# SvenGronauer/phoenix-drone-simulation

Measured on AMD Instinct MI355X. Metric: env-steps/sec, higher is better.
Workload: dtype f32; 1 GPU; DroneHoverSimpleEnv-v0, 1048576 envs per GPU lockstep, fp32, observation noise off, thrust noise 0, domain randomisation -1, auto-reset on, action ring [64,N,4] = hover+0.0 + 0.1*N(0,1); envs_per_gpu=1048576, obs_dim=42, bytes_per_env_step=346, parallelism=env-shard x1, no data-path collective

## Files before the change

phoenix-drone-simulation_amd/csrc/pds_api.hip:

```cpp
#include <hip/hip_runtime.h>

#include <cmath>
#include <cstdarg>
#include <cstdio>
#include <cstdlib>
#include <cstring>
#include <new>
#include <utility>
#include <vector>

#include "pds_reset.h"
#include "pds_collect_args.h"
#include "pds_evaluate_args.h"
#include "pds_evaluate_hist_args.h"
#include "pds_simopt.h"

namespace pds {

struct FieldArgs {
  DevState st;
  Consts k;
  void *user;
  long long n;
  int field;
  int task;
  int set;
// ... 182 lines not shown
  if (i >= n) return;
  const uint32_t c = st.ctr[i];
  if (ctr_oh(c) != 0u) return;
  const WaveClock ck = st.clk[i / kWave];
  const RngKey now{seed_lo, seed_hi, ck.x, ck.y};
  const float4 q0 = st.s0[i], q1 = st.s1[i], q2 = st.s2[i];
  const EnvRegs e{q0.x, q0.y, q0.z, q0.w, q1.x, q1.y, q1.z, q1.w, q2.x, q2.y, q2.z, q2.w};
  NoisyObs o;
  regen_kept_obs(k, (uint32_t)(env_id_base + (unsigned long long)i), now, ctr_step(c) == 0u, e, o);
  st.oh0[i] = make_float4(o.x, o.y, o.z, o.qx);
  st.oh1[i] = make_float4(o.qy, o.qz, o.qw, o.vx);
  st.oh2[i] = make_float2(o.vy, o.vz);
  st.ctr[i] = c | kCtrOhBit;
}


}

using namespace pds;

struct pds_handle {
  pds_config cfg;
  DevState st;
  Consts k;
  LaunchFlags flags;
  int force_tile;
  float2 *d_circle_ref;
  void *slab;
  float4 *lat_buf;
  unsigned long long *d_count;
  unsigned long long *d_stamps;
  void *eval_sink;
  int obs_dim;
  int num_cus;
  uint64_t tick;
  bool was_reset;
  bool after_evaluate;
  char err[512];
};

struct DeviceGuard {
  int prev = -1;
  bool switched = false;
  hipError_t err = hipSuccess;
  explicit DeviceGuard(int dev) {
    err = hipGetDevice(&prev);
    if (err == hipSuccess && prev != dev) {
      err = hipSetDevice(dev);
      switched = err == hipSuccess;
    }
  }
  ~DeviceGuard() {
// ... 13 lines not shown

static thread_local char g_create_err[512] = "";

#define PDS_HIP(h, call)                                                                        \
  do {                                                                                          \
    hipError_t e_ = (call);                                                                     \
    if (e_ != hipSuccess) return fail(h, PDS_EHIP, "%s failed: %s", #call, hipGetErrorString(e_)); \
  } while (0)

static int materialize_kept_obs(pds_handle *h, hipStream_t s) {
  if (!(h->flags.on && !h->flags.hold)) return PDS_OK;
  const long long n = h->cfg.num_envs;
  hipLaunchKernelGGL(pds::materialize_oh_kernel, dim3((unsigned)((n + kBlock - 1) / kBlock)), dim3(kBlock), 0, s, h->st, h->k, n,
                     (unsigned long long)h->cfg.env_id_base, (uint32_t)h->cfg.seed, (uint32_t)(h->cfg.seed >> 32));
  PDS_HIP(h, hipGetLastError());
  return PDS_OK;
}

extern "C" int pds_version(void) { return PDS_VERSION; }

extern "C" int pds_default_config(int task, pds_config *c) {
  if (!c || task < 0 || task > 2) return PDS_EINVAL;
  memset(c, 0, sizeof(*c));
  c->struct_size = (int32_t)sizeof(pds_config);
  c->task = task;
  c->num_envs = 1;
  c->env_id_base = 0;
  c->seed = 0;
  c->device = 0;
  c->use_motor_dynamics = 0;
// ... 189 lines not shown
  h->flags.ctrl = cfg->control_mode;
  h->flags.lat = lat_steps > 0;
  h->flags.hold = h->k.obs_rate != 1;
  h->flags.half_tile = false;
  if (const char *ft = getenv("PDS_FORCE_TILE")) h->force_tile = (ft[0] == 'h') ? 1 : ((ft[0] == 'f') ? 2 : 0);
  const size_t n = (size_t)cfg->num_envs;
  const size_t ntiles = (n + kWave - 1) / kWave;
  const LaunchFlags &f = h->flags;
  DeviceGuard guard(cfg->device);
  hipError_t e = guard.err;
  if (e == hipSuccess) {
    hipDeviceProp_t prop;
    e = hipGetDeviceProperties(&prop, cfg->device);
    h->num_cus = (e == hipSuccess && prop.multiProcessorCount > 0) ? prop.multiProcessorCount : 256;
  }
  std::vector<std::pair<void **, size_t>> req;
  auto alloc = [&](void **p, size_t bytes) { req.emplace_back(p, bytes); };
  alloc((void **)&h->st.s0, n * 16); alloc((void **)&h->st.s1, n * 16); alloc((void **)&h->st.s2, n * 16);
  alloc((void **)&h->st.hist[0], n * 16); alloc((void **)&h->st.hist[1], n * 16);
  alloc((void **)&h->st.ctr, n * 4);
  alloc((void **)&h->st.clk, ntiles * sizeof(WaveClock));
  alloc((void **)&h->d_count, 256);
  if (f.motor) alloc((void **)&h->st.mx, n * 16);
  if (f.dr) { alloc((void **)&h->st.par0, n * 16); alloc((void **)&h->st.par1, n * 8); }
  if (f.dr && f.motor) { alloc((void **)&h->st.mA, n * 16); alloc((void **)&h->st.mK, n * 16); }
  if (f.tn) alloc((void **)&h->st.ou, n * 16);
  if (f.on) {
    alloc((void **)&h->st.nz0, n * 16); alloc((void **)&h->st.nz1, n * 8);
    alloc((void **)&h->st.oh0, n * 16); alloc((void **)&h->st.oh1, n * 16); alloc((void **)&h->st.oh2, n * 8);
  }
// ... 69 lines not shown
  if (!h) return 0;
  DeviceGuard guard(h->cfg.device);
  WaveClock c;
  if (hipStreamSynchronize((hipStream_t)stream) == hipSuccess &&
      hipMemcpy(&c, h->st.clk, sizeof(c), hipMemcpyDeviceToHost) == hipSuccess)
    h->tick = ((uint64_t)c.y << 32) | c.x;
  return h->tick;
}

extern "C" int pds_set_tick(pds_handle *h, uint64_t tick) {
  if (!h) return PDS_EINVAL;
  DeviceGuard guard(h->cfg.device);
  PDS_HIP(h, guard.err);
  PDS_HIP(h, hipDeviceSynchronize());
  if (const int rc = materialize_kept_obs(h, 0)) return rc;
  const long long ntiles = (h->cfg.num_envs + kWave - 1) / kWave;
  hipLaunchKernelGGL(clock_fill_kernel, dim3((unsigned)((ntiles + 255) / 256)), dim3(256), 0, 0, h->st.clk, ntiles,
                     (unsigned long long)tick, 1);
  PDS_HIP(h, hipGetLastError());
  PDS_HIP(h, hipDeviceSynchronize());
  h->tick = tick;
  return PDS_OK;
}

extern "C" int pds_set_latency(pds_handle *h, double latency) {
  if (!h) return PDS_EINVAL;
  if (h->flags.ge && h->flags.ctrl != 0) return fail(h, PDS_EUNSUPPORTED, "use_latency with the ground-effect extension: control_mode PWM only");
  int steps = 0;
  if (!(latency < h->cfg.time_step)) {
    steps = (int)(latency / h->cfg.time_step);
    if (steps < 1) return fail(h, PDS_EINVAL, "latency %g: buf_size 0 (the reference asserts buf_size > 0)", latency);
    if (steps > kMaxLatSteps) return fail(h, PDS_EUNSUPPORTED, "latency %g s = %d steps (limit %d)", latency, steps, kMaxLatSteps);
  }
  DeviceGuard guard(h->cfg.device);
  PDS_HIP(h, guard.err);
  PDS_HIP(h, hipDeviceSynchronize());
  if (steps > 0) {
    const int rc = ensure_latency_buffer(h);
    if (rc != PDS_OK) return rc;
  }
  h->cfg.latency = latency;
  h->cfg.use_latency = steps > 0;
  h->flags.lat = steps > 0;
  set_latency_consts(h->k, steps, h->cfg.aggregate_phy_steps);
  if (steps > 0) {
    const long long n = h->cfg.num_envs;
    hipLaunchKernelGGL(latency_clear_kernel, dim3((unsigned)((n + 255) / 256)), dim3(256), 0, 0, h->st, n, kMaxLatSteps);
    PDS_HIP(h, hipGetLastError());
    PDS_HIP(h, hipDeviceSynchronize());
  }
  return PDS_OK;
}

extern "C" int pds_simopt_latency_steps(const pds_handle *h, double latency) {
  if (!h) return PDS_EINVAL;
// ... 16 lines not shown
  if (max_lat_steps > kMaxLatSteps)
    return fail(h, PDS_EUNSUPPORTED, "a candidate's latency is %d time steps (limit %d): nothing was evaluated", max_lat_steps,
                kMaxLatSteps);
  if (P < 1 || M < 1 || T < 2 || pre_steps < 0 || max_lat_steps < 0)
    return fail(h, PDS_EINVAL, "pds_simopt_evaluate: P %lld, M %lld, T %d, pre_steps %d, max_lat_steps %d", (long long)P,
                (long long)M, T, pre_steps, max_lat_steps);
  if (M > (1 << 24) || P > (1 << 24) || P * ((M + kWave - 1) / kWave) > (int64_t)1 << 32)
    return fail(h, PDS_EINVAL, "pds_simopt_evaluate: P %lld x M %lld is beyond one launch: shard the candidates", (long long)P,
                (long long)M);
  if (!d_params || !d_lat_steps || !d_actions || !d_obs || !d_loss || !d_score || (pre_steps > 0 && !d_pre_inputs))
    return fail(h, PDS_EINVAL, "pds_simopt_evaluate: null pointer");
  if (((uintptr_t)d_actions | (uintptr_t)d_obs | (uintptr_t)d_pre_inputs) & 15u)
    return fail(h, PDS_EINVAL, "pds_simopt_evaluate: the data set arrays must be 16-byte aligned");
  DeviceGuard guard(h->cfg.device);
  PDS_HIP(h, guard.err);
  SimoptArgs a;
  a.k = h->k;
  a.time_step = h->cfg.time_step;
  a.G = 9.81;
  a.gamma = gamma;
  a.params = d_params;
  a.lat_steps = d_lat_steps;
  a.acts = reinterpret_cast<const float4 *>(d_actions);
  a.obs = reinterpret_cast<const float4 *>(d_obs);
  a.pre = reinterpret_cast<const float4 *>(d_pre_inputs);
  a.P = (int)P; a.M = (int)M; a.T = T; a.pre_steps = pre_steps;
  a.loss = d_loss; a.score = d_score; a.sim_obs = d_sim_obs;
  launch_simopt(a, (hipStream_t)stream);
  PDS_HIP(h, hipGetLastError());
  return PDS_OK;
// ... 63 lines not shown
    else if (task == PDS_TASK_CIRCLE) launch_circle(kind, lf, grid, s, a);
    else launch_takeoff(kind, lf, grid, s, a);
  }
}

static int do_reset(pds_handle *h, const uint8_t *d_mask, const float *d_samples, float *d_obs, void *stream) {
  if (!h) return PDS_EINVAL;
  DeviceGuard guard(h->cfg.device);
  PDS_HIP(h, guard.err);
  if (d_mask != nullptr && h->after_evaluate)
    return fail(h, PDS_EINVAL, "pds_reset with a mask after pds_evaluate_policies: reset every env first (d_mask = NULL)");
  StepArgs a;
  base_args(h, a);
  a.mask = d_mask; a.samples = d_samples; a.obs = d_obs;
  const dim3 grid((unsigned)((a.n + kBlock - 1) / kBlock));
  if (d_mask != nullptr)
    if (const int rc = materialize_kept_obs(h, (hipStream_t)stream)) return rc;
  launch_family(h, kLaunchReset, h->flags, grid, (hipStream_t)stream, a);
  PDS_HIP(h, hipGetLastError());
  h->tick += 1;
  h->was_reset = true;
  h->after_evaluate = false;
  return PDS_OK;
}

extern "C" int pds_reset(pds_handle *h, const uint8_t *d_mask, float *d_obs, void *stream) {
  return do_reset(h, d_mask, nullptr, d_obs, stream);
}

extern "C" int pds_reset_from_samples(pds_handle *h, const uint8_t *d_mask, const float *d_samples,
                                      float *d_obs, void *stream) {
  if (h && !d_samples) return fail(h, PDS_EINVAL, "pds_reset_from_samples: d_samples is NULL");
  return do_reset(h, d_mask, d_samples, d_obs, stream);
}

static int check_step_pointers(pds_handle *h, const float *d_actions, float *d_obs, float *d_reward, uint8_t *d_terminated,
                               uint8_t *d_truncated, float *d_cost) {
// ... 13 lines not shown
  DeviceGuard guard(h->cfg.device);
  PDS_HIP(h, guard.err);
  StepArgs a;
  base_args(h, a);
  a.actions = reinterpret_cast<const float4 *>(d_actions);
  a.obs = d_obs; a.reward = d_reward; a.term = d_terminated; a.trunc = d_truncated; a.cost = d_cost;
  a.final_obs = d_final_obs;
  a.noise = d_variates;
  const dim3 grid((unsigned)((a.n + kBlock - 1) / kBlock));
  LaunchFlags lf = h->flags;
  const bool merged = !lf.on && !lf.lat && !(lf.motor && lf.dr) && h->cfg.task != PDS_TASK_TAKEOFF && h->cfg.auto_reset;
  const unsigned cus = (unsigned)h->num_cus;
  lf.half_tile = grid.x > (unsigned)kFullTileBlocksPerCU * cus * (256 / kBlock) && grid.x <= (merged ? 5u : 8u) * cus * (256 / kBlock);
  if (h->force_tile) lf.half_tile = h->force_tile == 1;
  if (lf.on || lf.lat) lf.half_tile = false;
  launch_family(h, kLaunchStep, lf, grid, (hipStream_t)stream, a);
  PDS_HIP(h, hipGetLastError());
  h->tick += 1;
  return PDS_OK;
}

extern "C" int pds_step(pds_handle *h, const float *d_actions, float *d_obs, float *d_reward,
                        uint8_t *d_terminated, uint8_t *d_truncated, float *d_cost, float *d_final_obs,
                        void *stream) {
  return pds_step_with_variates(h, d_actions, nullptr, d_obs, d_reward, d_terminated, d_truncated, d_cost,
                                d_final_obs, stream);
}

extern "C" int pds_step_k(pds_handle *h, int k_steps, const float *d_actions, float *d_obs, float *d_reward,
                          uint8_t *d_terminated, uint8_t *d_truncated, float *d_cost, float *d_final_obs, void *stream) {
  if (!h) return PDS_EINVAL;
  if (k_steps < 1) return fail(h, PDS_EINVAL, "pds_step_k: k_steps %d", k_steps);
// ... 9 lines not shown
    }
    return PDS_OK;
  }
  DeviceGuard guard(h->cfg.device);
  PDS_HIP(h, guard.err);
  StepArgs a;
  base_args(h, a);
  a.actions = reinterpret_cast<const float4 *>(d_actions);
  a.obs = d_obs; a.reward = d_reward; a.term = d_terminated; a.trunc = d_truncated; a.cost = d_cost;
  a.final_obs = d_final_obs;
  a.k_steps = k_steps;
  const dim3 grid((unsigned)((a.n + kBlock - 1) / kBlock));
  LaunchFlags lf = h->flags;
  lf.half_tile = false;
  if (const int rc = materialize_kept_obs(h, (hipStream_t)stream)) return rc;
  launch_family(h, kLaunchStepK, lf, grid, (hipStream_t)stream, a);
  PDS_HIP(h, hipGetLastError());
  h->tick += (uint64_t)k_steps;
  return PDS_OK;
}

extern "C" int pds_field_width(int field) {
  switch (field) {
    case PDS_F_POS: case PDS_F_RPY: case PDS_F_VEL: case PDS_F_OMEGA: case PDS_F_GYRO_BIAS: case PDS_F_GYRO_LPF: return 3;
    case PDS_F_QUAT: case PDS_F_MOTOR_X: case PDS_F_LAST_ACTION: case PDS_F_PREV_ACTION: case PDS_F_MOTOR_A:
    case PDS_F_MOTOR_K: case PDS_F_OU: return 4;
    case PDS_F_STEP_COUNT: case PDS_F_QUAT_SIGN: case PDS_F_REF_OFFSET: case PDS_F_ACTION_IDX: return 1;
    case PDS_F_PARAMS: return 6;
    case PDS_F_NOISY_OBS: return 10;
    case PDS_F_PID: return 12;
// ... 27 lines not shown
  ra.s.reward = d_rew_buf; ra.s.term = d_term_buf; ra.s.trunc = d_trunc_buf; ra.s.cost = d_cost_buf;
  ra.s.final_obs = nullptr;
  ra.s.k_steps = T;
  ra.pi = *pi;
  ra.mean = d_mean; ra.stdv = d_std; ra.eps = eps; ra.log_std = d_log_std;
  ra.seed = seed; ra.call_base = reinterpret_cast<const unsigned long long *>(d_call_base); ra.call_offset = call_offset;
  ra.deterministic = deterministic; ra.T = T;
  ra.act_buf = d_act_buf; ra.logp_buf = d_logp_buf;
  ra.ep_ret = d_ep_ret; ra.ep_len = d_ep_len; ra.stats = d_stats;
}
template <class Launch>
static int launch_rollout(pds_handle *h, const char *fn, int T, void *stream, Launch launch) {
  DeviceGuard guard(h->cfg.device);
  PDS_HIP(h, guard.err);
  if (const int rc = materialize_kept_obs(h, (hipStream_t)stream)) return rc;
  const dim3 grid((unsigned)((h->cfg.num_envs + kWave - 1) / kWave));
  if (!launch(grid, (hipStream_t)stream)) return fail(h, PDS_EHIP, "%s: its _supported() rule and the launchers disagree", fn);
  PDS_HIP(h, hipGetLastError());
  h->tick += (uint64_t)T;
  return PDS_OK;
}

extern "C" int pds_rollout(pds_handle *h, int T, const pds_mlp *pi, const pds_mlp *vf, const float *d_mean, const float *d_std,
                           float eps, const float *d_log_std, uint64_t seed, const uint64_t *d_call_base, uint64_t call_offset,
                           int deterministic, float *d_obs_buf, float *d_act_buf, float *d_logp_buf, float *d_val_buf,
                           float *d_rew_buf, uint8_t *d_term_buf, uint8_t *d_trunc_buf, float *d_cost_buf, float *d_fval_buf,
                           float *d_last_val, float *d_ep_ret, float *d_ep_len, float *d_stats, void *stream) {
  if (!h) return PDS_EINVAL;
  if (T < 1) return fail(h, PDS_EINVAL, "pds_rollout: T %d", T);
  const bool any_null = !pi || !vf || !d_log_std || !d_obs_buf || !d_act_buf || !d_logp_buf || !d_val_buf || !d_rew_buf ||
// ... 383 lines not shown
}

static int do_field(pds_handle *h, int field, void *d_ptr, int set, void *stream) {
  if (!h) return PDS_EINVAL;
  if (!d_ptr || pds_field_width(field) < 0) return fail(h, PDS_EINVAL, "bad field %d or NULL pointer", field);
  if (set && field == PDS_F_QUAT) return fail(h, PDS_EINVAL, "PDS_F_QUAT is derived (set PDS_F_RPY / PDS_F_QUAT_SIGN)");
  DeviceGuard guard(h->cfg.device);
  PDS_HIP(h, guard.err);
  FieldArgs a;
  memset(&a, 0, sizeof(a));
  a.st = h->st; a.k = h->k; a.user = d_ptr; a.n = h->cfg.num_envs; a.field = field; a.task = h->cfg.task; a.set = set;
  a.has_motor = h->flags.motor; a.has_dr = h->flags.dr; a.has_tn = h->flags.tn; a.has_on = h->flags.on; a.ctrl = h->flags.ctrl;
  a.regen_obs = h->flags.on && !h->flags.hold;
  if (set && field != PDS_F_NOISY_OBS)
    if (const int rc = materialize_kept_obs(h, (hipStream_t)stream)) return rc;
  a.env_id_base = (unsigned long long)h->cfg.env_id_base;
  a.seed_lo = (uint32_t)h->cfg.seed; a.seed_hi = (uint32_t)(h->cfg.seed >> 32);
  const dim3 grid((unsigned)((a.n + kBlock - 1) / kBlock));
  hipLaunchKernelGGL(field_kernel, grid, dim3(kBlock), 0, (hipStream_t)stream, a);
  PDS_HIP(h, hipGetLastError());
  if (set && !h->after_evaluate) h->was_reset = true;
  return PDS_OK;
}

extern "C" int pds_count_nonfinite(pds_handle *h, int64_t *count, void *stream) {
  if (!h || !count) return PDS_EINVAL;
  DeviceGuard guard(h->cfg.device);
  PDS_HIP(h, guard.err);
  hipStream_t s = (hipStream_t)stream;
  PDS_HIP(h, hipMemsetAsync(h->d_count, 0, sizeof(*h->d_count), s));
  const long long n = h->cfg.num_envs;
  hipLaunchKernelGGL(nonfinite_kernel, dim3((unsigned)((n + 255) / 256)), dim3(256), 0, s, h->st, n, h->d_count);
  PDS_HIP(h, hipGetLastError());
  unsigned long long host = 0;
  PDS_HIP(h, hipMemcpyAsync(&host, h->d_count, sizeof(host), hipMemcpyDeviceToHost, s));
  PDS_HIP(h, hipStreamSynchronize(s));
  *count = (int64_t)host;
  return PDS_OK;
}

extern "C" int pds_get_state(pds_handle *h, int field, void *d_out, void *stream) { return do_field(h, field, d_out, 0, stream); }
extern "C" int pds_set_state(pds_handle *h, int field, const void *d_in, void *stream) { return do_field(h, field, const_cast<void *>(d_in), 1, stream); }

template <int ROUNDS>
// ... 77 lines not shown
```

phoenix-drone-simulation_amd/csrc/pds_step.h:

```cpp
#pragma once
#include <type_traits>
#include "pds_reset.h"
#include "pds_physics.h"

namespace pds {

template <int D>
constexpr int tile_stride() {
  return (D % 8 == 0) ? D + 4 : D;
}

template <int HW>
constexpr int park_stride() {
  return (HW % 4 == 0) ? ((HW / 4) % 2 == 1 ? HW : HW + 4) : (HW % 2 == 1 ? HW : HW + 1);
}

template <int N>
PDS_DEV void lds_store_row(float *dst, const float *src) {
  static_assert(N % 4 == 0, "float4 rows");
#pragma unroll
  for (int j = 0; j < N / 4; ++j)
    reinterpret_cast<float4 *>(dst)[j] = make_float4(src[4 * j], src[4 * j + 1], src[4 * j + 2], src[4 * j + 3]);
}

template <class V>
constexpr bool heavy_variant() { return V::MOTOR || V::DR || V::TN || V::ON || V::CTRL != 0 || V::LAT; }

template <class V>
constexpr bool saddr_variant() { return heavy_variant<V>(); }
template <class V>
constexpr bool park_variant() { return heavy_variant<V>(); }
template <class V>
using Idx = EnvIdxT<saddr_variant<V>()>;

template <class V>
constexpr bool regen_obs_variant() { return V::ON && !V::HOLD && !V::OH_STORED; }
template <class V>
constexpr bool flags_oh_variant() { return V::ON && !V::HOLD && V::OH_STORED; }

template <int D, int TR, bool SADDR>
PDS_DEV void flush_tile(const float *tile, float *gdst, int rows, int lane) {
  constexpr int TS = tile_stride<D>();
  const bool fast = rows == TR && (reinterpret_cast<uintptr_t>(gdst) & 15u) == 0;
  if constexpr (TS == D) {
    if (fast) {
      constexpr int NV = TR * D / 4;
      const float4 *src = reinterpret_cast<const float4 *>(tile);
      float4 *dst = reinterpret_cast<float4 *>(gdst);
// ... 130 lines not shown
  if constexpr (regen_obs_variant<V>()) {
    const uint32_t env_id = (uint32_t)(a.env_id_base + (unsigned long long)ix.wb) + ix.lc;
    regen_kept_obs(a.k, env_id, rk, ctr_step(S.ctr) == 0u, S.e, S.oh);
    const bool stored = ctr_oh(S.ctr) != 0u;
    if (__ballot(stored) != 0ull) {
      if (stored) {
        const float4 o0 = *at(a.st.oh0, ix), o1 = *at(a.st.oh1, ix);
        const float2 o2 = *at(a.st.oh2, ix);
        S.oh = NoisyObs{o0.x, o0.y, o0.z, o0.w, o1.x, o1.y, o1.z, o1.w, o2.x, o2.y};
      }
    }
  }
}

template <class V>
PDS_DEV void store_state(const StepArgs &a, const Idx<V> i_, int new_parity, const EnvState &S, bool both) {
  const EnvRegs &e = S.e;
  Idx<V> i = fresh<3>(i_);
  st_store4(at(a.st.s0, i), make_float4(e.px, e.py, e.pz, e.vx));
  st_store4(at(a.st.s1, i), make_float4(e.vy, e.vz, e.roll, e.pitch));
  st_store4(at(a.st.s2, i), make_float4(e.yaw, e.wx, e.wy, e.wz));
  st_store4(at(a.st.hist[new_parity], i), S.h1);
  *at(a.st.ctr, i) = flags_oh_variant<V>() ? (S.ctr | kCtrOhBit) : S.ctr;
  if (V::MOTOR) *at(a.st.mx, i) = make_float4(S.xm[0], S.xm[1], S.xm[2], S.xm[3]);
  if (V::TN) *at(a.st.ou, i) = make_float4(S.ns.ou[0], S.ns.ou[1], S.ns.ou[2], S.ns.ou[3]);
  if (V::CTRL >= 1) {
    *at(a.st.pid0, i) = make_float4(S.ps.rate_int[0], S.ps.rate_int[1], S.ps.rate_int[2], S.ps.rate_err[0]);
    *at(a.st.pid1, i) = make_float2(S.ps.rate_err[1], S.ps.rate_err[2]);
  }
  if (V::CTRL == 2) {
    *at(a.st.pid2, i) = make_float4(S.ps.att_int[0], S.ps.att_int[1], S.ps.att_int[2], S.ps.att_err[0]);
    *at(a.st.pid3, i) = make_float2(S.ps.att_err[1], S.ps.att_err[2]);
  }
  if (V::ON) {
    *at(a.st.nz0, i) = make_float4(S.ns.bias[0], S.ns.bias[1], S.ns.bias[2], S.ns.lpf[0]);
    *at(a.st.nz1, i) = make_float2(S.ns.lpf[1], S.ns.lpf[2]);
// ... 189 lines not shown
constexpr int inline_envs() {
  return (STORE || V::TASK != PDS_TASK_HOVER) ? inline_envs_per_pass<V>() : PDS_INLINE_ENVS_KSTEP;
}
template <class V>
constexpr int scratch_stride() { return (variates_floats<V>() + 3) / 4; }
template <class V>
constexpr bool four_block_variant() {
  return regen_obs_variant<V>() && V::TASK == PDS_TASK_HOVER && !(V::MOTOR && V::DR) && V::CTRL == 0 && !V::LAT;
}

struct StepOut {
  float reward;
  bool done, trunc;
};

template <class V, int TR, int RM, bool STORE>
PDS_DEV bool step_once(const StepArgs &a, const long long o1, const RngKey &rk, int parity, const float2 *ref_lds,
                       float *tile, float *park, uint32_t *queue, U4 *scratch, int lane, long long wave_base, const Idx<V> ix,
                       bool active, const float4 act, EnvState &S, int &qcount, float *fin_lds, StepOut *so
#ifdef PDS_STAMPS
                       , unsigned long long *stamp_
#endif
) {
  constexpr int TASK = V::TASK;
  constexpr int D = V::D;
  constexpr int O = V::O;
  constexpr int TS = tile_stride<D>();
  constexpr bool VEC = (TS != D) && TR == kWave;
  static_assert(RM != RM_MERGED || (!V::ON && !V::LAT), "merged reset: variants without observation noise / latency");
  static_assert(RM != RM_INLINE || TR == kWave, "inline reset: full tile only");
  static_assert(RM != RM_DEFERRED || STORE, "deferred drain: the state must be in HBM before it");
// ... 18 lines not shown
  const int phase1 = (TASK == PDS_TASK_CIRCLE) ? ((phase + 1 == k.ref_points) ? 0 : phase + 1) : 0;
  int ref_offset = 0;
  if (TASK == PDS_TASK_CIRCLE && !k.reset_dist) ref_offset = (int)circle_ref_offset(ctr, k.ref_points);

  float4 pa1 = h2, pa2 = h1;
  if (V::LAT) {
    if (step == 0) {
      if (k.lat_own1 == 1) { pa1 = act; pa2 = act; }
    } else if (step == 1) {
      if (k.lat_own2 == 2) pa1 = act;
      else if (k.lat_own2 == 1) pa1 = h1;
    }
  }

  Quat q = quat_from_euler(e.roll, e.pitch, e.yaw);
  {
    float tx, ty, tz;
    target_at<TASK>(k, ref_lds, target_index<TASK>(step, k.agg, phase), tx, ty, tz);
    if (V::ON) {
      put_noisy_half<TASK, O + 4, VEC1>(row, S.oh, ns.lpf, h1, tx, ty, tz, pa1);
    } else {
      Quat qk = q;
      if (ctr_sign(ctr)) { qk.x = -q.x; qk.y = -q.y; qk.z = -q.z; qk.w = -q.w; }
      put_obs_half<TASK, O + 4, VEC1>(row, e, qk, h1, tx, ty, tz, pa1);
    }
  }

  float *xm = S.xm;
  NoisyObs held = S.oh;
  uint32_t lat_idx = ctr_lat(ctr);
  const float inv_m = fast_rcp(par.m), inv_Jx = fast_rcp(par.Jx), inv_Jy = fast_rcp(par.Jy), inv_Jz = fast_rcp(par.Jz);
  for (int sub = 0; sub < k.agg; ++sub) {
    SubNoise sn;
    if (V::TN || V::ON) sub_noise<V>(a, rk, env_id, ix, sub, sn);
    float av[4] = {act.x, act.y, act.z, act.w};
    if (V::LAT) {
      float4 *slot = a.st.lat + (long long)lat_idx * a.n + ix.global();
      const float4 d = *slot;
      if (active) *slot = act;
      lat_idx = (lat_idx + 1u == (uint32_t)k.lat_steps) ? 0u : lat_idx + 1u;
      av[0] = d.x; av[1] = d.y; av[2] = d.z; av[3] = d.w;
    }
    float f[4], pwmv[4];
    if (V::CTRL == 0) {
      PDS_PWM_FROM_ACTION()
    } else {
      control_pwm<V::CTRL>(k.dt_nom, e, av, ps, pwmv);
    }
    PDS_MOTOR_THRUST(V::MOTOR, V::TN, ns.ou, sn.ou)
    PDS_RIGID_BODY_SUBSTEP(V::GE, !V::ON || sub + 1 < k.agg)
    if (V::ON) {
      if (!V::HOLD) {
        gyro_update(k, e, sn.bias_z, sn.rw_z, sn.to_z, ns);
      } else {
        const int it = step * k.agg + sub;
        const bool fresh = (it % k.obs_rate) == 0;
        NoisyObs cand;
        sensor_observe(k, e, sn.full, ns, cand);
        held.x = fresh ? cand.x : held.x; held.y = fresh ? cand.y : held.y; held.z = fresh ? cand.z : held.z;
        held.qx = fresh ? cand.qx : held.qx; held.qy = fresh ? cand.qy : held.qy; held.qz = fresh ? cand.qz : held.qz;
        held.qw = fresh ? cand.qw : held.qw;
        held.vx = fresh ? cand.vx : held.vx; held.vy = fresh ? cand.vy : held.vy; held.vz = fresh ? cand.vz : held.vz;
      }
    }
// ... 87 lines not shown
      reset_in_registers<V>(a, rk, ref_lds, queue, count, need_reset, pos, lane, wave_base, ref_offset, scratch, e, q,
                            u0, mxr, par, S.ctr);
      if (need_reset) {
        was_reset = true;
        S.h1 = u0; S.h2 = u0;
        xm[0] = mxr.x; xm[1] = mxr.y; xm[2] = mxr.z; xm[3] = mxr.w;
#pragma unroll
        for (int j = 0; j < 3; ++j) { ps.rate_int[j] = ps.rate_err[j] = ps.att_int[j] = ps.att_err[j] = 0.f; }
      }
    }
  }

  {
  const StepArgs &a = reload_args<102, heavy_variant<V>()>(a_in, (int)o1);
  const Consts &k = a.k;
  if (active) {
    if constexpr (STORE && RM != RM_INLINE) store_state<V>(a, ix, parity ^ 1, S, was_reset);
    if constexpr (STORE && RM == RM_INLINE) {
      if (!need_reset) store_state<V>(a, ix, parity ^ 1, S, false);
    }
    const Idx<V> jx = fresh<5>(ix);
    nt_store(at(a.reward + o1, jx), reward);
    nt_store(at(a.cost + o1, jx), cost);
    nt_store(at(a.term + o1, jx), (uint8_t)(done ? 1 : 0));
    nt_store(at(a.trunc + o1, jx), (uint8_t)(trunc ? 1 : 0));
  }
  PDS_STAMP(4);
  const long long rem = a.n - wave_base;
#pragma unroll
  for (int pass = 0; pass < kWave / TR; ++pass) {
    if (TR != kWave) {
      if ((lane / TR) == pass) {
// ... 233 lines not shown
#else
#define PDS_STAMP_ARG
#define PDS_STAMP_DECL
#define PDS_STAMP_FLUSH do { } while (0)
#endif

#define PDS_CLOCK_TO_KEY(clk, rk, parity)                                  \
  rk.tick_lo = (uint32_t)__builtin_amdgcn_readfirstlane((int)clk.x);       \
  rk.tick_hi = (uint32_t)__builtin_amdgcn_readfirstlane((int)clk.y);       \
  parity = __builtin_amdgcn_readfirstlane((int)clk.z) & 1;
#define PDS_NEXT_TICK(rk, parity) \
  parity ^= 1;                    \
  rk.tick_lo += 1u;               \
  if (rk.tick_lo == 0u) rk.tick_hi += 1u;

template <class V, int TR>
__global__ __launch_bounds__(kBlock, (PDS_MIN_WAVES) * (256 / kBlock)) void step_kernel(const StepArgs a) {
  PDS_STAMP_DECL
  prefetch_kernargs();
  constexpr int RM = merged_reset_variant<V, TR>() ? RM_MERGED : (inline_reset_single_step<V, TR>() ? RM_INLINE : RM_DEFERRED);
  PDS_WAVE_SETUP(V, TR, RM, true)
  Loaded cur;
  load_env<V>(a, ix, t, cur);
  __builtin_amdgcn_sched_barrier(0);
  PDS_STAMP(1);
  PDS_STAMP_WAIT(2);
  RngKey rk{a.seed_lo, a.seed_hi, 0u, 0u};
  int parity;
  PDS_CLOCK_TO_KEY(cur.clk, rk, parity)
  EnvState S;
  unpack_state<V>(a.k, cur, parity, S);
  init_kept_obs<V>(a, rk, ix, S);
  int qcount = 0;
  step_once<V, TR, RM, true>(a, 0ll, rk, parity, ref_lds, tile, park, queue, scratch, lane, wave_base, ix, active, cur.act, S, qcount, nullptr, nullptr PDS_STAMP_ARG);
  if (RM == RM_DEFERRED && qcount > 0) {
    const float own_w[3] = {S.e.wx, S.e.wy, S.e.wz};
    drain_reset_queue<V>(reload_args<104, heavy_variant<V>()>(a), rk, ref_lds, queue, qcount, lane, wave_base, tile, own_w, S.ns.bias);
  }
  PDS_STAMP(6);
  advance_clock(reload_args<105, heavy_variant<V>()>(a).st.clk, t, rk, parity ^ 1, 1u, lane);
  PDS_STAMP_FLUSH;
}

#ifndef PDS_STEPK_MIN_WAVES_OF
#define PDS_STEPK_MIN_WAVES_OF(V) 3
#endif
template <class V_>
__global__ __launch_bounds__(kBlock, (PDS_STEPK_MIN_WAVES_OF(V_)) * (256 / kBlock)) void step_k_kernel(const StepArgs a) {
  using W = std::conditional_t<regen_obs_variant<V_>(), StoredOh<V_>, V_>;
  constexpr int TR = kWave;
  constexpr int RM = merged_reset_variant<W>() ? RM_MERGED : RM_INLINE;
#ifdef PDS_STAMPS
  unsigned long long stamp_[kStampSlots];
#endif
  prefetch_kernargs();
  PDS_WAVE_SETUP(W, TR, RM, false)
// ... 23 lines not shown
  }
  const StepArgs &az = reload_args<107, heavy_variant<W>()>(a);
  if (active) store_state<W>(az, ix, parity, S, true);
  advance_clock(az.st.clk, t, rk0, parity, (uint32_t)K, lane);
}

template <class V>
inline void launch_variant(int kind, bool half_tile, dim3 grid, hipStream_t s, const StepArgs &a) {
  if (kind == kLaunchReset) {
    if constexpr (!V::GE && !V::TN && V::CTRL == 0 && !V::HOLD) hipLaunchKernelGGL((reset_kernel<V>), grid, dim3(kBlock), 0, s, a);
    else abort();
  } else if (kind == kLaunchStepK) {
    if constexpr (step_k_rule(V::CTRL, V::GE, V::HOLD)) hipLaunchKernelGGL((step_k_kernel<V>), grid, dim3(kBlock), 0, s, a);
    else abort();
  } else {
    if constexpr (!V::ON && !V::LAT) {
      if (half_tile) {
        hipLaunchKernelGGL((step_kernel<V, kHalfTileRows>), grid, dim3(kBlock), 0, s, a);
        return;
      }
    }
    hipLaunchKernelGGL((step_kernel<V, kWave>), grid, dim3(kBlock), 0, s, a);
  }
}

template <int TASK, int CTRL, bool LAT, bool HOLD, bool MOTOR, bool DR, bool GE, bool TN, bool ON>
struct MakeVariant {
  using type = Variant<TASK, MOTOR, DR, GE, TN, ON, CTRL, LAT, HOLD>;
};

// ... 80 lines not shown
```

phoenix-drone-simulation_amd/csrc/pds_types.h:

```cpp
#pragma once
#include <hip/hip_runtime.h>
#include <stddef.h>
#include <stdint.h>

#include "../../include/pds.h"
#include "pds_device.h"

namespace pds {

#ifndef PDS_BLOCK
#define PDS_BLOCK 256
#endif
constexpr int kBlock = PDS_BLOCK;
constexpr int kWave = 64;
constexpr int kHalfTileRows = 32;
constexpr int kFullTileBlocksPerCU = 3;
constexpr int kQueueCap = 64;
constexpr int kRefPoints = 300;
constexpr int kStaggerBytes = 4352;

constexpr int kStampSlots = 10;
constexpr int kMaxLatSteps = PDS_MAX_LATENCY_STEPS;

PDS_DEV uint32_t ctr_pack(uint32_t step, uint32_t sign, uint32_t off, uint32_t lat_idx = 0u) {
  return step | (sign << 16) | (off << 17) | (lat_idx << 26);
}
PDS_DEV uint32_t ctr_step(uint32_t c) { return c & 0xFFFFu; }
PDS_DEV uint32_t ctr_sign(uint32_t c) { return (c >> 16) & 1u; }
PDS_DEV uint32_t ctr_off(uint32_t c) { return (c >> 17) & 0x1FFu; }
PDS_DEV uint32_t ctr_lat(uint32_t c) { return (c >> 26) & 0x7u; }
constexpr uint32_t kCtrOhBit = 1u << 29;
PDS_DEV uint32_t ctr_oh(uint32_t c) { return (c >> 29) & 1u; }
PDS_DEV uint32_t circle_ref_offset(uint32_t c, int ref_points) {
  const int d = (int)ctr_off(c) - (int)(ctr_step(c) % (uint32_t)ref_points);
  return (uint32_t)(d < 0 ? d + ref_points : d);
}

template <bool SADDR>
struct EnvIdxT {
  long long wb;
  uint32_t lc;
  PDS_DEV long long global() const { return wb + (long long)lc; }
};
template <>
struct EnvIdxT<false> {
  long long wb;
  uint32_t lc;
// ... 193 lines not shown
  if (TASK == PDS_TASK_CIRCLE) return phase;
  if (TASK == PDS_TASK_TAKEOFF) return min(step * agg, kRefPoints - 1);
  return 0;
}

struct LaunchFlags {
  bool motor, dr, ge, tn, on;
  int ctrl;
  bool lat;
  bool hold;
  bool half_tile;
};
constexpr bool inline_single_step_rule(int task, bool on, bool lat, int ctrl) {
  return (on || lat) && task != PDS_TASK_TAKEOFF && !(task == PDS_TASK_CIRCLE && (lat || ctrl != 0));
}
enum LaunchKind { kLaunchStep = 0, kLaunchStepK = 1, kLaunchReset = 2 };
constexpr bool step_k_rule(int ctrl, bool ge, bool hold) { return ctrl == 0 || (!ge && !hold); }
inline bool step_k_supported(const LaunchFlags &f) { return step_k_rule(f.ctrl, f.ge, f.hold); }
struct RolloutArgs {
  StepArgs s;
  pds_mlp pi, vf;
  const float *mean, *stdv;
  float eps;
  const float *log_std;
  unsigned long long seed;
  const unsigned long long *call_base;
  unsigned long long call_offset;
  int deterministic, T;
  const float *obs0;
  float *act_buf, *logp_buf, *val_buf, *fval_buf, *last_val;
  float *ep_ret, *ep_len, *stats;
// ... 67 lines not shown
```

Measured before the change: 18.93 billion env-steps/s.

## Store env state every other step and recompute the lagging step on load

```diff
diff --git a/phoenix-drone-simulation_amd/csrc/pds_api.hip b/phoenix-drone-simulation_amd/csrc/pds_api.hip
--- a/phoenix-drone-simulation_amd/csrc/pds_api.hip
+++ b/phoenix-drone-simulation_amd/csrc/pds_api.hip
@@ -10,6 +10,7 @@
 #include <vector>
 
 #include "pds_reset.h"
+#include "pds_physics.h"
 #include "pds_collect_args.h"
 #include "pds_evaluate_args.h"
 #include "pds_evaluate_hist_args.h"
@@ -222,6 +223,34 @@
   st.ctr[i] = c | kCtrOhBit;
 }
 
+__global__ __launch_bounds__(kBlock) void materialize_state_kernel(DevState st, Consts k, long long n, int ge) {
+  const long long i = (long long)blockIdx.x * kBlock + threadIdx.x;
+  if (i >= n) return;
+  const uint32_t c = st.ctr[i];
+  if (ctr_behind(c) == 0u) return;
+  const int parity = (int)(st.clk[i / kWave].z & 1u);
+  const float4 q0 = st.s0[i], q1 = st.s1[i], q2 = st.s2[i];
+  const float4 act = st.hist[parity][i];
+  EnvRegs e{q0.x, q0.y, q0.z, q0.w, q1.x, q1.y, q1.z, q1.w, q2.x, q2.y, q2.z, q2.w};
+  Params par;
+  default_params(k, par);
+  float xm_[4] = {0.f, 0.f, 0.f, 0.f}, ou_[4] = {0.f, 0.f, 0.f, 0.f};
+  float *xm = xm_;
+  Quat q = quat_from_euler(e.roll, e.pitch, e.yaw);
+  const float inv_m = fast_rcp(par.m), inv_Jx = fast_rcp(par.Jx), inv_Jy = fast_rcp(par.Jy), inv_Jz = fast_rcp(par.Jz);
+  for (int sub = 0; sub < k.agg; ++sub) {
+    float av[4] = {act.x, act.y, act.z, act.w};
+    float f[4], pwmv[4];
+    PDS_PWM_FROM_ACTION()
+    PDS_MOTOR_THRUST(false, false, ou_, ou_)
+    PDS_RIGID_BODY_SUBSTEP(ge != 0, true)
+  }
+  st.s0[i] = make_float4(e.px, e.py, e.pz, e.vx);
+  st.s1[i] = make_float4(e.vy, e.vz, e.roll, e.pitch);
+  st.s2[i] = make_float4(e.yaw, e.wx, e.wy, e.wz);
+  st.ctr[i] = c & ~kCtrBehindBit;
+}
+
 
 }
 
@@ -233,6 +262,7 @@
   Consts k;
   LaunchFlags flags;
   int force_tile;
+  bool store_every_step;
   float2 *d_circle_ref;
   void *slab;
   float4 *lat_buf;
@@ -244,6 +274,8 @@
   uint64_t tick;
   bool was_reset;
   bool after_evaluate;
+  bool state_maybe_behind;
+  bool step_captured;
   char err[512];
 };
 
@@ -287,6 +319,21 @@
   hipLaunchKernelGGL(pds::materialize_oh_kernel, dim3((unsigned)((n + kBlock - 1) / kBlock)), dim3(kBlock), 0, s, h->st, h->k, n,
                      (unsigned long long)h->cfg.env_id_base, (uint32_t)h->cfg.seed, (uint32_t)(h->cfg.seed >> 32));
   PDS_HIP(h, hipGetLastError());
+  return PDS_OK;
+}
+
+static bool skips_state(const pds_handle *h) {
+  const LaunchFlags &f = h->flags;
+  return PDS_STATE_EVERY_OTHER_STEP != 0 && !h->store_every_step && !f.motor && !f.dr && !f.tn && !f.on && f.ctrl == 0 && !f.lat;
+}
+
+static int materialize_state(pds_handle *h, hipStream_t s) {
+  if (!h->state_maybe_behind && !h->step_captured) return PDS_OK;
+  const long long n = h->cfg.num_envs;
+  hipLaunchKernelGGL(pds::materialize_state_kernel, dim3((unsigned)((n + kBlock - 1) / kBlock)), dim3(kBlock), 0, s, h->st, h->k, n,
+                     h->flags.ge ? 1 : 0);
+  PDS_HIP(h, hipGetLastError());
+  h->state_maybe_behind = false;
   return PDS_OK;
 }
 
@@ -506,6 +553,11 @@
     e = hipGetDeviceProperties(&prop, cfg->device);
     h->num_cus = (e == hipSuccess && prop.multiProcessorCount > 0) ? prop.multiProcessorCount : 256;
   }
+  {
+    const size_t blocks = (n + kBlock - 1) / kBlock;
+    h->store_every_step = blocks <= (size_t)kFullTileBlocksPerCU * (size_t)h->num_cus * (256 / kBlock);
+    if (const char *es = getenv("PDS_STATE_EVERY_STEP")) h->store_every_step = es[0] == '1';
+  }
   std::vector<std::pair<void **, size_t>> req;
   auto alloc = [&](void **p, size_t bytes) { req.emplace_back(p, bytes); };
   alloc((void **)&h->st.s0, n * 16); alloc((void **)&h->st.s1, n * 16); alloc((void **)&h->st.s2, n * 16);
@@ -605,6 +657,7 @@
   PDS_HIP(h, guard.err);
   PDS_HIP(h, hipDeviceSynchronize());
   if (const int rc = materialize_kept_obs(h, 0)) return rc;
+  if (const int rc = materialize_state(h, 0)) return rc;
   const long long ntiles = (h->cfg.num_envs + kWave - 1) / kWave;
   hipLaunchKernelGGL(clock_fill_kernel, dim3((unsigned)((ntiles + 255) / 256)), dim3(256), 0, 0, h->st.clk, ntiles,
                      (unsigned long long)tick, 1);
@@ -630,6 +683,7 @@
     const int rc = ensure_latency_buffer(h);
     if (rc != PDS_OK) return rc;
   }
+  if (const int rc = materialize_state(h, 0)) return rc;
   h->cfg.latency = latency;
   h->cfg.use_latency = steps > 0;
   h->flags.lat = steps > 0;
@@ -676,6 +730,7 @@
     return fail(h, PDS_EINVAL, "pds_simopt_evaluate: the data set arrays must be 16-byte aligned");
   DeviceGuard guard(h->cfg.device);
   PDS_HIP(h, guard.err);
+  if (const int rc = materialize_state(h, (hipStream_t)stream)) return rc;
   SimoptArgs a;
   a.k = h->k;
   a.time_step = h->cfg.time_step;
@@ -769,13 +824,16 @@
   base_args(h, a);
   a.mask = d_mask; a.samples = d_samples; a.obs = d_obs;
   const dim3 grid((unsigned)((a.n + kBlock - 1) / kBlock));
-  if (d_mask != nullptr)
+  if (d_mask != nullptr) {
     if (const int rc = materialize_kept_obs(h, (hipStream_t)stream)) return rc;
+    if (const int rc = materialize_state(h, (hipStream_t)stream)) return rc;
+  }
   launch_family(h, kLaunchReset, h->flags, grid, (hipStream_t)stream, a);
   PDS_HIP(h, hipGetLastError());
   h->tick += 1;
   h->was_reset = true;
   h->after_evaluate = false;
+  if (d_mask == nullptr) h->state_maybe_behind = false;
   return PDS_OK;
 }
 
@@ -819,8 +877,14 @@
   lf.half_tile = grid.x > (unsigned)kFullTileBlocksPerCU * cus * (256 / kBlock) && grid.x <= (merged ? 5u : 8u) * cus * (256 / kBlock);
   if (h->force_tile) lf.half_tile = h->force_tile == 1;
   if (lf.on || lf.lat) lf.half_tile = false;
-  launch_family(h, kLaunchStep, lf, grid, (hipStream_t)stream, a);
+  launch_family(h, h->store_every_step ? kLaunchStepStoreAll : kLaunchStep, lf, grid, (hipStream_t)stream, a);
   PDS_HIP(h, hipGetLastError());
+  if (skips_state(h)) {
+    h->state_maybe_behind = true;
+    hipStreamCaptureStatus cs = hipStreamCaptureStatusNone;
+    if (hipStreamIsCapturing((hipStream_t)stream, &cs) != hipSuccess) (void)hipGetLastError();
+    else if (cs != hipStreamCaptureStatusNone) h->step_captured = true;
+  }
   h->tick += 1;
   return PDS_OK;
 }
@@ -860,6 +924,7 @@
   LaunchFlags lf = h->flags;
   lf.half_tile = false;
   if (const int rc = materialize_kept_obs(h, (hipStream_t)stream)) return rc;
+  if (const int rc = materialize_state(h, (hipStream_t)stream)) return rc;
   launch_family(h, kLaunchStepK, lf, grid, (hipStream_t)stream, a);
   PDS_HIP(h, hipGetLastError());
   h->tick += (uint64_t)k_steps;
@@ -917,6 +982,7 @@
   DeviceGuard guard(h->cfg.device);
   PDS_HIP(h, guard.err);
   if (const int rc = materialize_kept_obs(h, (hipStream_t)stream)) return rc;
+  if (const int rc = materialize_state(h, (hipStream_t)stream)) return rc;
   const dim3 grid((unsigned)((h->cfg.num_envs + kWave - 1) / kWave));
   if (!launch(grid, (hipStream_t)stream)) return fail(h, PDS_EHIP, "%s: its _supported() rule and the launchers disagree", fn);
   PDS_HIP(h, hipGetLastError());
@@ -1330,6 +1396,7 @@
   a.regen_obs = h->flags.on && !h->flags.hold;
   if (set && field != PDS_F_NOISY_OBS)
     if (const int rc = materialize_kept_obs(h, (hipStream_t)stream)) return rc;
+  if (const int rc = materialize_state(h, (hipStream_t)stream)) return rc;
   a.env_id_base = (unsigned long long)h->cfg.env_id_base;
   a.seed_lo = (uint32_t)h->cfg.seed; a.seed_hi = (uint32_t)(h->cfg.seed >> 32);
   const dim3 grid((unsigned)((a.n + kBlock - 1) / kBlock));
@@ -1344,6 +1411,7 @@
   DeviceGuard guard(h->cfg.device);
   PDS_HIP(h, guard.err);
   hipStream_t s = (hipStream_t)stream;
+  if (const int rc = materialize_state(h, s)) return rc;
   PDS_HIP(h, hipMemsetAsync(h->d_count, 0, sizeof(*h->d_count), s));
   const long long n = h->cfg.num_envs;
   hipLaunchKernelGGL(nonfinite_kernel, dim3((unsigned)((n + 255) / 256)), dim3(256), 0, s, h->st, n, h->d_count);
diff --git a/phoenix-drone-simulation_amd/csrc/pds_step.h b/phoenix-drone-simulation_amd/csrc/pds_step.h
--- a/phoenix-drone-simulation_amd/csrc/pds_step.h
+++ b/phoenix-drone-simulation_amd/csrc/pds_step.h
@@ -32,6 +32,9 @@
 constexpr bool park_variant() { return heavy_variant<V>(); }
 template <class V>
 using Idx = EnvIdxT<saddr_variant<V>()>;
+
+template <class V>
+constexpr bool skip_state_variant() { return PDS_STATE_EVERY_OTHER_STEP != 0 && !heavy_variant<V>(); }
 
 template <class V>
 constexpr bool regen_obs_variant() { return V::ON && !V::HOLD && !V::OH_STORED; }
@@ -192,12 +195,14 @@
 }
 
 template <class V>
-PDS_DEV void store_state(const StepArgs &a, const Idx<V> i_, int new_parity, const EnvState &S, bool both) {
+PDS_DEV void store_state(const StepArgs &a, const Idx<V> i_, int new_parity, const EnvState &S, bool both, bool behind = false) {
   const EnvRegs &e = S.e;
   Idx<V> i = fresh<3>(i_);
-  st_store4(at(a.st.s0, i), make_float4(e.px, e.py, e.pz, e.vx));
-  st_store4(at(a.st.s1, i), make_float4(e.vy, e.vz, e.roll, e.pitch));
-  st_store4(at(a.st.s2, i), make_float4(e.yaw, e.wx, e.wy, e.wz));
+  if (!behind) {
+    st_store4(at(a.st.s0, i), make_float4(e.px, e.py, e.pz, e.vx));
+    st_store4(at(a.st.s1, i), make_float4(e.vy, e.vz, e.roll, e.pitch));
+    st_store4(at(a.st.s2, i), make_float4(e.yaw, e.wx, e.wy, e.wz));
+  }
   st_store4(at(a.st.hist[new_parity], i), S.h1);
   *at(a.st.ctr, i) = flags_oh_variant<V>() ? (S.ctr | kCtrOhBit) : S.ctr;
   if (V::MOTOR) *at(a.st.mx, i) = make_float4(S.xm[0], S.xm[1], S.xm[2], S.xm[3]);
@@ -417,7 +422,7 @@
   bool done, trunc;
 };
 
-template <class V, int TR, int RM, bool STORE>
+template <class V, int TR, int RM, bool STORE, bool SKIPSTATE = false>
 PDS_DEV bool step_once(const StepArgs &a, const long long o1, const RngKey &rk, int parity, const float2 *ref_lds,
                        float *tile, float *park, uint32_t *queue, U4 *scratch, int lane, long long wave_base, const Idx<V> ix,
                        bool active, const float4 act, EnvState &S, int &qcount, float *fin_lds, StepOut *so
@@ -466,7 +471,7 @@
   }
 
   Quat q = quat_from_euler(e.roll, e.pitch, e.yaw);
-  {
+  auto first_half = [&]() {
     float tx, ty, tz;
     target_at<TASK>(k, ref_lds, target_index<TASK>(step, k.agg, phase), tx, ty, tz);
     if (V::ON) {
@@ -476,16 +481,30 @@
       if (ctr_sign(ctr)) { qk.x = -q.x; qk.y = -q.y; qk.z = -q.z; qk.w = -q.w; }
       put_obs_half<TASK, O + 4, VEC1>(row, e, qk, h1, tx, ty, tz, pa1);
     }
+  };
+  constexpr bool SKIP = SKIPSTATE;
+  static_assert(!SKIP || (STORE && skip_state_variant<V>() && RM != RM_INLINE), "state every other step: the lean single-step kernels");
+  const bool behind = SKIP && ctr_behind(ctr) != 0u;
+  int sub_first = 0;
+  float4 ua = h1;
+  if constexpr (SKIP) {
+    if (__ballot(behind) != 0ull) sub_first = -k.agg;
+  } else {
+    first_half();
   }
 
   float *xm = S.xm;
   NoisyObs held = S.oh;
   uint32_t lat_idx = ctr_lat(ctr);
   const float inv_m = fast_rcp(par.m), inv_Jx = fast_rcp(par.Jx), inv_Jy = fast_rcp(par.Jy), inv_Jz = fast_rcp(par.Jz);
-  for (int sub = 0; sub < k.agg; ++sub) {
+  for (int sub = sub_first; sub < k.agg; ++sub) {
+    if constexpr (SKIP) {
+      if (sub == 0) { first_half(); ua = act; }
+    }
     SubNoise sn;
     if (V::TN || V::ON) sub_noise<V>(a, rk, env_id, ix, sub, sn);
     float av[4] = {act.x, act.y, act.z, act.w};
+    if constexpr (SKIP) { av[0] = ua.x; av[1] = ua.y; av[2] = ua.z; av[3] = ua.w; }
     if (V::LAT) {
       float4 *slot = a.st.lat + (long long)lat_idx * a.n + ix.global();
       const float4 d = *slot;
@@ -500,6 +519,10 @@
       control_pwm<V::CTRL>(k.dt_nom, e, av, ps, pwmv);
     }
     PDS_MOTOR_THRUST(V::MOTOR, V::TN, ns.ou, sn.ou)
+    if constexpr (SKIP) {
+      if (sub >= 0 || behind) { PDS_RIGID_BODY_SUBSTEP(V::GE, true) }
+      continue;
+    }
     PDS_RIGID_BODY_SUBSTEP(V::GE, !V::ON || sub + 1 < k.agg)
     if (V::ON) {
       if (!V::HOLD) {
@@ -617,8 +640,15 @@
   {
   const StepArgs &a = reload_args<102, heavy_variant<V>()>(a_in, (int)o1);
   const Consts &k = a.k;
+  const unsigned long long fresh_lanes = SKIP ? __ballot(was_reset) : 0ull;
   if (active) {
-    if constexpr (STORE && RM != RM_INLINE) store_state<V>(a, ix, parity ^ 1, S, was_reset);
+    if constexpr (SKIP) {
+      const bool line_mate = ((fresh_lanes >> (lane & ~7)) & 0xFFull) != 0ull;
+      const bool skip = (rk.tick_lo & 1u) != 0u && !behind && !line_mate;
+      if (skip) S.ctr |= kCtrBehindBit;
+      store_state<V>(a, ix, parity ^ 1, S, was_reset, skip);
+    }
+    if constexpr (STORE && RM != RM_INLINE && !SKIP) store_state<V>(a, ix, parity ^ 1, S, was_reset);
     if constexpr (STORE && RM == RM_INLINE) {
       if (!need_reset) store_state<V>(a, ix, parity ^ 1, S, false);
     }
@@ -882,32 +912,40 @@
   rk.tick_lo += 1u;               \
   if (rk.tick_lo == 0u) rk.tick_hi += 1u;
 
+#define PDS_STEP_KERNEL_BODY(SKIPSTATE_) \
+  PDS_STAMP_DECL \
+  prefetch_kernargs(); \
+  constexpr int RM = merged_reset_variant<V, TR>() ? RM_MERGED : (inline_reset_single_step<V, TR>() ? RM_INLINE : RM_DEFERRED); \
+  PDS_WAVE_SETUP(V, TR, RM, true) \
+  Loaded cur; \
+  load_env<V>(a, ix, t, cur); \
+  __builtin_amdgcn_sched_barrier(0); \
+  PDS_STAMP(1); \
+  PDS_STAMP_WAIT(2); \
+  RngKey rk{a.seed_lo, a.seed_hi, 0u, 0u}; \
+  int parity; \
+  PDS_CLOCK_TO_KEY(cur.clk, rk, parity) \
+  EnvState S; \
+  unpack_state<V>(a.k, cur, parity, S); \
+  init_kept_obs<V>(a, rk, ix, S); \
+  int qcount = 0; \
+  step_once<V, TR, RM, true, SKIPSTATE_>(a, 0ll, rk, parity, ref_lds, tile, park, queue, scratch, lane, wave_base, ix, active, cur.act, S, qcount, nullptr, nullptr PDS_STAMP_ARG); \
+  if (RM == RM_DEFERRED && qcount > 0) { \
+    const float own_w[3] = {S.e.wx, S.e.wy, S.e.wz}; \
+    drain_reset_queue<V>(reload_args<104, heavy_variant<V>()>(a), rk, ref_lds, queue, qcount, lane, wave_base, tile, own_w, S.ns.bias); \
+  } \
+  PDS_STAMP(6); \
+  advance_clock(reload_args<105, heavy_variant<V>()>(a).st.clk, t, rk, parity ^ 1, 1u, lane); \
+  PDS_STAMP_FLUSH;
+
 template <class V, int TR>
 __global__ __launch_bounds__(kBlock, (PDS_MIN_WAVES) * (256 / kBlock)) void step_kernel(const StepArgs a) {
-  PDS_STAMP_DECL
-  prefetch_kernargs();
-  constexpr int RM = merged_reset_variant<V, TR>() ? RM_MERGED : (inline_reset_single_step<V, TR>() ? RM_INLINE : RM_DEFERRED);
-  PDS_WAVE_SETUP(V, TR, RM, true)
-  Loaded cur;
-  load_env<V>(a, ix, t, cur);
-  __builtin_amdgcn_sched_barrier(0);
-  PDS_STAMP(1);
-  PDS_STAMP_WAIT(2);
-  RngKey rk{a.seed_lo, a.seed_hi, 0u, 0u};
-  int parity;
-  PDS_CLOCK_TO_KEY(cur.clk, rk, parity)
-  EnvState S;
-  unpack_state<V>(a.k, cur, parity, S);
-  init_kept_obs<V>(a, rk, ix, S);
-  int qcount = 0;
-  step_once<V, TR, RM, true>(a, 0ll, rk, parity, ref_lds, tile, park, queue, scratch, lane, wave_base, ix, active, cur.act, S, qcount, nullptr, nullptr PDS_STAMP_ARG);
-  if (RM == RM_DEFERRED && qcount > 0) {
-    const float own_w[3] = {S.e.wx, S.e.wy, S.e.wz};
-    drain_reset_queue<V>(reload_args<104, heavy_variant<V>()>(a), rk, ref_lds, queue, qcount, lane, wave_base, tile, own_w, S.ns.bias);
-  }
-  PDS_STAMP(6);
-  advance_clock(reload_args<105, heavy_variant<V>()>(a).st.clk, t, rk, parity ^ 1, 1u, lane);
-  PDS_STAMP_FLUSH;
+  PDS_STEP_KERNEL_BODY(false)
+}
+template <int TR, class V>
+__global__ __launch_bounds__(kBlock, (PDS_MIN_WAVES) * (256 / kBlock)) void skip_step_kernel(const StepArgs a) {
+  static_assert(skip_state_variant<V>(), "the lean variants");
+  PDS_STEP_KERNEL_BODY(true)
 }
 
 #ifndef PDS_STEPK_MIN_WAVES_OF
@@ -961,6 +999,13 @@
     if constexpr (step_k_rule(V::CTRL, V::GE, V::HOLD)) hipLaunchKernelGGL((step_k_kernel<V>), grid, dim3(kBlock), 0, s, a);
     else abort();
   } else {
+    if constexpr (skip_state_variant<V>()) {
+      if (kind == kLaunchStep) {
+        if (half_tile) hipLaunchKernelGGL((skip_step_kernel<kHalfTileRows, V>), grid, dim3(kBlock), 0, s, a);
+        else hipLaunchKernelGGL((skip_step_kernel<kWave, V>), grid, dim3(kBlock), 0, s, a);
+        return;
+      }
+    }
     if constexpr (!V::ON && !V::LAT) {
       if (half_tile) {
         hipLaunchKernelGGL((step_kernel<V, kHalfTileRows>), grid, dim3(kBlock), 0, s, a);
diff --git a/phoenix-drone-simulation_amd/csrc/pds_types.h b/phoenix-drone-simulation_amd/csrc/pds_types.h
--- a/phoenix-drone-simulation_amd/csrc/pds_types.h
+++ b/phoenix-drone-simulation_amd/csrc/pds_types.h
@@ -31,6 +31,11 @@
 PDS_DEV uint32_t ctr_lat(uint32_t c) { return (c >> 26) & 0x7u; }
 constexpr uint32_t kCtrOhBit = 1u << 29;
 PDS_DEV uint32_t ctr_oh(uint32_t c) { return (c >> 29) & 1u; }
+#ifndef PDS_STATE_EVERY_OTHER_STEP
+#define PDS_STATE_EVERY_OTHER_STEP 1
+#endif
+constexpr uint32_t kCtrBehindBit = 1u << 30;
+PDS_DEV uint32_t ctr_behind(uint32_t c) { return (c >> 30) & 1u; }
 PDS_DEV uint32_t circle_ref_offset(uint32_t c, int ref_points) {
   const int d = (int)ctr_off(c) - (int)(ctr_step(c) % (uint32_t)ref_points);
   return (uint32_t)(d < 0 ? d + ref_points : d);
@@ -254,7 +259,7 @@
 constexpr bool inline_single_step_rule(int task, bool on, bool lat, int ctrl) {
   return (on || lat) && task != PDS_TASK_TAKEOFF && !(task == PDS_TASK_CIRCLE && (lat || ctrl != 0));
 }
-enum LaunchKind { kLaunchStep = 0, kLaunchStepK = 1, kLaunchReset = 2 };
+enum LaunchKind { kLaunchStep = 0, kLaunchStepK = 1, kLaunchReset = 2, kLaunchStepStoreAll = 3 };
 constexpr bool step_k_rule(int ctrl, bool ge, bool hold) { return ctrl == 0 || (!ge && !hold); }
 inline bool step_k_supported(const LaunchFlags &f) { return step_k_rule(f.ctrl, f.ge, f.hold); }
 struct RolloutArgs {
```

After: 19.56 billion env-steps/s (median of 6 runs). +3.3%, better.
